# Lapin0t/py-swirld

Hardware: AMD Instinct MI355X
Metric: events/sec through divide_rounds+decide_fame (higher is better)
Workload: dtype int32; 1 GPU; 256 members, 1000000 events, uniform-gossip hashgraph, one batch divide_rounds + decide_fame per step; members=256, events=1000000, seed=3, parallelism=replicas x1 (no data-path collective); the one-hashgraph split is `value_strong`, rounds=284, new_c_last_step=280

## Files before the change

### py-swirld_amd/csrc/swirld_hip.hip

```cpp
#include <hip/hip_runtime.h>

#include <algorithm>
#include <atomic>
#include <chrono>
#include <cstdarg>
#include <cstdio>
#include <cstring>
#include <initializer_list>
#include <string>
#include <thread>
#include <type_traits>
#include <vector>

#include "../../include/swirld_hip.h"
#include "entry_plan.h"
#include "owned.h"
#include "kernels.hip.h"
#define SW_PROV_ROWS 16
#define SW_RANGE_SLOTS 16
#include "crypto.hip.h"
#include "validate.hip.h"
#include "pack.hip.h"
#include "sign.hip.h"
#include "data.hip.h"
#include "exact.hip.h"
#include "batch.hip.h"
#include "ingest.hip.h"
#include "resolve.hip.h"
#include "gossip.hip.h"
#include "walk.hip.h"
#include "wire.hip.h"
#include "turn.hip.h"
#include "consensus.hip.h"
#include "votes.hip.h"

namespace {

std::string g_create_error;

using owned::DBuf;
using owned::Event;
using owned::Pinned;
using owned::Stream;

struct PinnedVec {
    Pinned<int32_t> buf;
    size_t n = 0;
    size_t size() const { return n; }
    int32_t* data() { return buf.p; }
    int32_t& operator[](size_t i) { return buf.p[i]; }
    void clear() { n = 0; }
    bool resize(size_t m) {
        if (m > buf.cap) {
            Pinned<int32_t> q;
            if (!q.reserve(std::max(m, buf.cap + buf.cap / 2 + 4096))) return false;
            if (n) memcpy(q.p, buf.p, n * sizeof(int32_t));
            buf = std::move(q);
        }
        n = m;
        return true;
    }
};

}

struct VmTable {
    bool active = false;
    char* base = nullptr;
    size_t va_bytes = 0, chunk = 0;
    std::vector<hipMemGenericAllocationHandle_t> handle;
// ... 80 lines not shown
    Event ev_payload;
    bool payload_pending = false;
    std::vector<int32_t> seq_h;
    Pinned<SmallRec> h_small;
    Event ev_small;
    bool small_pending = false;
    Pinned<char> h_pin;
    int max_height = 0;
    int64_t N = 0, cap = 0, divided = 0;
    struct IngestState {
        DBuf<int32_t> d_tab;
        DBuf<int32_t> d_hist;
        DBuf<int32_t> d_ht_stat;
        std::vector<int32_t> stage;
        Event ev_ht;
        bool ht_pending = false;
        int64_t ht_first = 0, ht_K = 0;
        int64_t ht_dev_upto = 0;
        int64_t dev_batches = 0, dev_events = 0, fallback = 0, host_ht = 0;
        void rewind() {}
        void reset() { ht_pending = false; ht_dev_upto = 0; }
    } ing;
    struct IdState {
        DBuf<unsigned char> d_id;
        DBuf<int32_t> d_idtab;
        int idtab_log = 0;
        int64_t n_ids = 0;
        DBuf<int32_t> d_idflag;
        DBuf<unsigned char> d_pl;
        DBuf<unsigned char> d_pl_in;
        Pinned<int32_t> h_plcnt;
        int64_t pl_calls = 0, pl_waves = 0, pl_accepted = 0, pl_rebuilds = 0;
        double pl_ms[4] = {0, 0, 0, 0};
        void rewind() {}
        void reset() { n_ids = 0; }
    } ids;
    struct ExportState {
        DBuf<int32_t> d;
        DBuf<unsigned char> d_out;
        int64_t calls = 0, events = 0;
        double ms[2] = {0, 0};
        int lanes = 16;
    } xp;
    struct VotesState {
        DBuf<unsigned char> d_sched, d_plan, d_work, d_out;
        int sched_calls = -1;
        std::vector<unsigned char> sched_stage, plan_stage;
        DBuf<unsigned long long> d_cnt;
        int64_t calls = 0, rows = 0, entries = 0;
        double ms[2] = {0, 0};
        void rewind() { sched_calls = -1; }
        void reset() {}
    } votes;
    struct WalkState {
        DBuf<int32_t> d;
        DBuf<unsigned> d_bits;
        DBuf<int32_t> d_q;
        DBuf<int32_t> d_list;
        DBuf<int32_t> d_trunk;
        DBuf<int32_t> d_children;
        int64_t trunk_N = -1;
        int threads = 1024;
        int64_t calls = 0, events = 0, levels = 0;
        double ms[3] = {0, 0, 0};
        void rewind() {}
        void reset() { trunk_N = -1; }
    } walk;
    struct ConsensusState {
        DBuf<int32_t> d_rr;
        DBuf<double> d_cts;
        DBuf<int32_t> d_tx;
        int64_t tx_len = 0;
        DBuf<int32_t> d_ordpos;
        DBuf<unsigned char> d_out;
        int64_t record_calls = 0, recorded = 0, export_calls = 0, exported = 0;
        void rewind() { tx_len = 0; }
        void reset() {}
    } cons;
    struct ValidateState {
        std::vector<uint8_t> keys, usable;
        DBuf<unsigned char> d_keys;
        DBuf<unsigned char> d_tab;
        DBuf<unsigned char> d_in;
        int64_t calls = 0, events = 0, accepted = 0, builds = 0;
        double ms[2] = {0, 0};
    } val;
    struct PackState {
        std::string mod = "swirld", qual = "Event";
        bool hdr_stale = true;
        std::vector<uint8_t> hdr;
        DBuf<unsigned char> d_hdr;
        DBuf<unsigned char> d;
        DBuf<unsigned char> d_in;
        DBuf<unsigned char> d_out;
        Pinned<int32_t> h_cnt;
        int64_t calls = 0, events = 0, bytes = 0;
        double ms[2] = {0, 0};
    } pack;
    struct DataState {
        DBuf<unsigned char> d_arena;
        DBuf<long long> d_off;
        DBuf<unsigned char> d_none;
        int64_t n_data = 0;
        int64_t used = 0;
        DBuf<unsigned char> d;
        DBuf<unsigned char> d_in;
// ... 86 lines not shown
    int64_t stage_calls = 0;
    DBuf<unsigned long long> d_dbg;
    DBuf<unsigned long long> d_dbg_blk;
    int64_t dbg_iter_base = 0;
    int dbg_minor = 1;
    DBuf<unsigned char> d_small;
    Event ev_aux_done, ev_cs_done, ev_main_mark, ev_bounds, ev_loop_done;
    std::vector<int32_t> divided_cnt;
    std::vector<int32_t> bounds_stage;
    DBuf<int32_t> d_evalround, d_evalpos, d_lo_r, d_cur, d_unres, d_lo_next, d_pos_next, d_farslot, d_force, d_cand, d_gallop;
    DBuf<u64> d_Mb;
    DBuf<int32_t> d_Pc;
    DBuf<int32_t> d_rsc;
    DBuf<u64> d_found64;
    DBuf<unsigned char> d_rb;
    Pinned<unsigned char> h_rb_all;
    std::vector<Event> rb_events;
    RState* d_state = nullptr;
    int* d_flow_err = nullptr;
    struct { int32_t* p = nullptr; } d_front;
    int32_t* d_treecnt = nullptr;
    unsigned* d_prov = nullptr;
    FameCounters* d_fc = nullptr;
    unsigned char* h_rb = nullptr;
    int gate_lag = 0, gate_step = 1;
    int gated = 1;
    int shot_pct = 100, shot_extra = 2;
    size_t rb_bytes = 0;
    Pinned<unsigned char> h_fame;
    std::vector<int32_t> front;
    std::vector<int32_t> front_dev;
    std::vector<int32_t> lo0_h;
    std::vector<unsigned char> cons_h;
    int sw_dirty_from = 1;

    int skip = 1;
    int gallop_after = 2;
    int elect_impl = 1;
    int elect_cg = 128;
    int K = 28;
    int MCAP = 0;
    int NEARCAP = 0;
    int BATCH = 24;
    int cansee_impl = 6;
    int ring_H_req = 0;
    int flow_cfg = 1;
    int tally_impl = 1;
    bool tally_auto = true;
    bool K_auto = true;
    int K_flat = 28;
    int eval_src = 0;
    int band_blocks = 512;
    int fin_blocks = 1024;
    int mid_pct = 0;
    int fin_band = 1;
    int band_fast = 1;
    int tally_filter = 0;
    int tally_pf = 1;

    struct GraphKey { int Rcap; int64_t N; void* lo; void* L; void* chain; void* S; void* round; int K, tally_impl, BATCH, MCAP, variant; };
    bool use_graph = true;
    hipGraph_t loop_graph[4] = {nullptr, nullptr, nullptr, nullptr};
    hipGraphExec_t loop_exec[4] = {nullptr, nullptr, nullptr, nullptr};
    int graph_big = 64;
    GraphKey loop_key{};
    int64_t stat_iters = 0, stat_events = 0;
    int64_t gstat_iters = 0, gstat_events = 0;

    bool profiling = false;
    sw_timings tm{};
    sw_counters ctr{};
    std::vector<Event> ev_pool;
    size_t ev_used = 0;
    PinnedVec transactions;
    std::vector<int32_t> ord_pos;
    std::vector<unsigned char> sig_h;
    std::vector<int32_t> chain_start_h, chain_ev_h;
    DBuf<int32_t> d_q, d_acc_ev, d_acc_ri, d_sorted, d_hostflag;
    DBuf<int32_t> d_ord_rounds, d_fwm, d_ordat, d_rowsum, d_grp;
    DBuf<long long> d_oblk;
    Pinned<char> h_ord;
    std::vector<Event> ord_events;
    Pinned<int32_t> h_ord_stage;
    DBuf<int32_t> d_big_ri, d_sk_ev;
    DBuf<long long> d_big_off;
    DBuf<double> d_sk_ts;
    DBuf<u64> d_sk_k8;
    DBuf<int32_t> d_seg;
    DBuf<int32_t> d_fd;
    DBuf<unsigned char> d_white;
    DBuf<double> d_ts;
    DBuf<double> d_tch;
    DBuf<int> d_err;
    DBuf<u64> d_flow_dbg;
};

namespace {

int fail(sw_ctx* c, int code, const char* fmt, ...) {
    char buf[512];
    va_list ap;
    va_start(ap, fmt);
    vsnprintf(buf, sizeof buf, fmt, ap);
    va_end(ap);
    if (c) c->err = buf; else g_create_error = buf;
    return code;
// ... 776 lines not shown
    for (int g = 0; g < 4; ++g) {
        if (kGraphSizes[g] <= 0) continue;
        while (left >= kGraphSizes[g]) {
            if (!c->loop_exec[g]) {
                HIPCHK(c, hipStreamBeginCapture(c->stream, hipStreamCaptureModeThreadLocal));
                const int64_t launches_before = c->ctr.kernel_launches;
                for (int it = 0; it < kGraphSizes[g]; ++it) enqueue_iteration<NW>(c, it & 1, nullptr);
                c->ctr.kernel_launches = launches_before;
                HIPCHK(c, hipStreamEndCapture(c->stream, &c->loop_graph[g]));
                HIPCHK(c, hipGraphInstantiate(&c->loop_exec[g], c->loop_graph[g], nullptr, nullptr, 0));
            }
            HIPCHK(c, hipGraphLaunch(c->loop_exec[g], c->stream));
            c->ctr.kernel_launches += 2 * kGraphSizes[g];
            left -= kGraphSizes[g];
        }
    }
    return SW_OK;
}

template <int NW>
int launch_finalize(sw_ctx* c, hipStream_t ax, int64_t first, int64_t K, int R, int blocks) {
    const int np = c->npad;
    if (K <= 0) return SW_OK;
    if (!c->fin_band) {
        hipLaunchKernelGGL(k_finalize_events<NW>, dim3((unsigned)std::min<int64_t>((K + 3) / 4, blocks)), dim3(256), 0, ax, (const int*)c->d_L.p,
                           (const int*)c->d_cr.p, (const int*)c->d_lo.p, R, (int)first, (int)K, c->d_round.p, c->d_S.p, np);
        c->ctr.kernel_launches++;
        return SW_OK;
    }
    if (!c->d_fin.p) {
        CHK(dgrow(c, c->d_fin, 4, 0));
        HIPCHK(c, hipMemset(c->d_fin.p, 0, 16));
    }
    HIPCHK(c, hipMemsetAsync(c->d_fin.p, 0, sizeof(unsigned), ax));
    hipLaunchKernelGGL(k_finalize_check, dim3((unsigned)((K + 255) / 256)), dim3(256), 0, ax, (const int*)c->d_cr.p, (const int*)c->d_lo.p, R,
                       (int)first, (int)K, (const int*)c->d_round.p, np, c->d_finlist.p, c->d_fin.p);
    hipLaunchKernelGGL(k_finalize_listed<NW>, dim3((unsigned)std::min<int64_t>((K + 3) / 4, std::min(blocks, 1024))), dim3(256), 0, ax, (const int*)c->d_L.p,
                       (const int*)c->d_cr.p, (const int*)c->d_lo.p, R, (const int*)c->d_finlist.p, c->d_fin.p, c->d_round.p, c->d_S.p, np);
    c->ctr.kernel_launches += 2;
    return SW_OK;
}

inline int predict_shot(const sw_ctx* c, int64_t n_new_events, bool gated = false) {
    int shot = std::min<int64_t>(c->BATCH, 2 + (n_new_events / (12 * (int64_t)c->n) + 1) * 2);
    const int64_t si = gated ? c->gstat_iters : c->stat_iters, se = gated ? c->gstat_events : c->stat_events;
    if (si > 0 && se > 0) {
        const double pred = (double)si / (double)se * (double)n_new_events;
        shot = std::max(2, (int)(pred * c->shot_pct / 100.0) + c->shot_extra);
    }
    return std::min(shot, 4096) & ~1;
}

template <int NW>
int launch_voter_masks(sw_ctx* c, int r0, int R, hipStream_t strm) {
    const int np = c->npad;
    if (R > c->Sw_rows) {
        int nr = c->Sw_rows ? c->Sw_rows : 256;
        while (nr < R) nr *= 2;
        u64* q = nullptr;
        hipError_t e = hipMalloc((void**)&q, (size_t)nr * np * NW * sizeof(u64));
        if (e != hipSuccess) return fail(c, SW_ENOMEM, "hipMalloc(Sw) failed: %s", hipGetErrorString(e));
        poison(q, (size_t)nr * np * NW * sizeof(u64));
        HIPCHK(c, hipStreamSynchronize(c->stream_aux));
        if (c->Sw_rows && c->d_Sw.p)
            HIPCHK(c, hipMemcpy(q, c->d_Sw.p, (size_t)c->Sw_rows * np * NW * sizeof(u64), hipMemcpyDeviceToDevice));
        c->d_Sw.adopt(q, (size_t)nr * np * NW);
        c->Sw_rows = nr;
    }
    r0 = std::max(1, r0);
    if (R <= r0) return SW_OK;
    const uint32_t tot2 = 2u * c->tot;
    const int total = (R - r0) * np;
    if (c->unit_stake && c->tally_impl >= 1)
        hipLaunchKernelGGL(k_voter_masks_bits<NW>, dim3((total + 3) / 4), dim3(256), 0, strm,
                           (const int*)c->d_wit.p, (const int*)c->d_L.p, (const int*)c->d_lo.p, (const uint32_t*)c->d_S.p,
                           tot2, r0, R, np, (uint32_t*)c->d_Sw.p, c->d_fc);
    else if (c->unit_stake)
        hipLaunchKernelGGL((k_voter_masks<NW, true>), dim3((total + 3) / 4), dim3(256), 0, strm,
                           (const int*)c->d_wit.p, (const int*)c->d_L.p, (const int*)c->d_lo.p, (const u64*)c->d_S.p,
                           (const uint32_t*)c->d_stake.p, tot2, r0, R, np, c->d_Sw.p, c->d_fc);
    else
        hipLaunchKernelGGL((k_voter_masks<NW, false>), dim3((total + 3) / 4), dim3(256), 0, strm,
                           (const int*)c->d_wit.p, (const int*)c->d_L.p, (const int*)c->d_lo.p, (const u64*)c->d_S.p,
                           (const uint32_t*)c->d_stake.p, tot2, r0, R, np, c->d_Sw.p, c->d_fc);
    c->ctr.kernel_launches++;
    return SW_OK;
}

struct EdgeHeights {
    std::vector<int64_t> start;
    std::vector<std::vector<int32_t>> h;
    int32_t at(int64_t e) const {
        for (size_t i = 0; i < start.size(); ++i)
            if (e >= start[i] && e < start[i] + (int64_t)h[i].size()) return h[i][(size_t)(e - start[i])];
        return 0;
    }
};

void height_span(const sw_ctx* c, int64_t a, int64_t b, int* hmin, int* hmax, const EdgeHeights& edge) {
    int lo = 0x7fffffff, hi = -1;
    int64_t e = a;
    const int64_t have = (int64_t)c->ht.size();
    while (e < b) {
        if ((e & 4095) == 0 && e + 4096 <= b) {
            lo = std::min(lo, c->blk_hmin[e >> 12]);
            hi = std::max(hi, c->blk_hmax[e >> 12]);
            e += 4096;
        } else {
            const int32_t h = e < have ? c->ht[e] : edge.at(e);
            lo = std::min(lo, h);
            hi = std::max(hi, h);
            ++e;
        }
    }
    *hmin = lo;
    *hmax = hi;
}

int heights_for_spans(sw_ctx* c, const std::vector<int64_t>& cut, EdgeHeights& edge) {
    CHK(heights_ready(c));
    const int64_t have = (int64_t)c->sp.size();
    if (have >= c->N) return SW_OK;
    if (c->ing.ht_dev_upto < c->N) return ensure_dag_h(c);
    for (size_t i = 0; i < cut.size(); ++i) {
        const int64_t x = cut[i];
        const int64_t a = std::max<int64_t>(x & ~(int64_t)4095, have), b = std::min<int64_t>((x | (int64_t)4095) + 1, c->N);
        if ((x & 4095) == 0 || b <= a) continue;
        edge.start.push_back(a);
        edge.h.emplace_back((size_t)(b - a));
        HIPCHK(c, hipMemcpyAsync(edge.h.back().data(), c->d_ht.p + a, (size_t)(b - a) * sizeof(int32_t), hipMemcpyDeviceToHost, c->stream));
    }
    HIPCHK(c, hipStreamSynchronize(c->stream));
    return SW_OK;
}

struct StageClock {
    bool on;
    std::chrono::steady_clock::time_point last;
    explicit StageClock(bool on_) : on(on_) { if (on) last = std::chrono::steady_clock::now(); }
    void mark(double* acc) {
        if (!on) return;
        const auto now = std::chrono::steady_clock::now();
        *acc += std::chrono::duration<double, std::micro>(now - last).count();
        last = now;
    }
};


struct DeferredTail {
    bool armed;
    int i, r_start, R;
    int64_t a0, k0;
    hipEvent_t loop_done;
};

struct DivideCall {
    const int64_t first, K;
    std::vector<int64_t> cut;
    int S = 0;
    bool flow = false;
    bool preswept = false;
    bool gated = false;
    std::vector<int> hmins, nlevs;
    bool bounds_pending = false;
    std::vector<int32_t> clen_prev, clen;
    int64_t fin_from = 0;
    DeferredTail tail{};
    StageClock clk;
    Span sp_total, sp_rl;
    hipEvent_t cs_t0 = nullptr, cs_t1 = nullptr, fin_t0 = nullptr;
    float tally_ms = 0.f;
    int tally_launches = 0;
    std::vector<Span> cansee_spans;
    DivideCall(const sw_ctx* c, int64_t first_, int64_t K_) : first(first_), K(K_), clk(c->debug_timing) {}
};

LoopGate* loop_gate(sw_ctx* c) { return reinterpret_cast<LoopGate*>(c->d_rb.p + SW_GATE_OFF); }

void plan_cuts(const sw_ctx* c, DivideCall& d) {
    const int64_t first = d.first, K = d.K;
    std::vector<int64_t>& cut = d.cut;
    cut.assign(1, first);
    if (const char* cs_ = getenv("SW_CUTS"); cs_ && K >= 65536) {
        for (const char* q = cs_; *q;) {
            char* end = nullptr;
            const double f = strtod(q, &end);
            if (end == q) break;
            const int64_t bnd = ((first + (int64_t)(f * (double)K)) >> 12) << 12;
            if (bnd > cut.back() && bnd < first + K) cut.push_back(bnd);
            q = *end ? end + 1 : end;
        }
    } else if (K >= 65536 && c->pipe > 1) {
        const int64_t head = K / 16;
        const int P = c->pipe;
        double w[SW_PROV_ROWS], tot = 0.0;
        for (int s_ = 0; s_ < P; ++s_) { w[s_] = P < 4 ? 1.0 : (s_ == 0 ? 0.5 : s_ == 1 ? 0.9 : s_ == 2 ? 1.2 : 1.0); tot += w[s_]; }
        double acc = 0.0;
        for (int s_ = 0; s_ < P; ++s_) {
            const int64_t at = head + (int64_t)((double)(K - head) * (acc / tot));
            acc += w[s_];
            const int64_t bnd = ((first + at) >> 12) << 12;
            if (bnd > cut.back() && bnd < first + K) cut.push_back(bnd);
        }
    }
    cut.push_back(first + K);
    d.S = (int)cut.size() - 1;
    d.flow = c->cansee_impl >= 6;
}

void choose_tally(sw_ctx* c, const DivideCall& d) {
    if (!c->tally_auto || !c->unit_stake) return;
    int impl = 1;
    if (c->npad == 256 && c->n > 200 && d.K >= 65536) {
        int32_t lo_ = 0x7fffffff, hi_ = 0;
        for (int m = 0; m < c->n; ++m) { lo_ = std::min(lo_, c->nev[m]); hi_ = std::max(hi_, c->nev[m]); }
// ... 184 lines not shown
    int r_start = 0x7fffffff;
    bool row0_dirty = false;
    std::copy(c->bounds_stage.begin() + (size_t)(i + 1) * np, c->bounds_stage.begin() + (size_t)(i + 2) * np, d.clen.begin());
    for (int m = 0; m < c->n; ++m) {
        if (d.clen[m] > d.clen_prev[m]) {
            if (c->front[m] < 0) {
                c->lo0_h[m] = c->first_ev[m];
                c->front[m] = 0;
                row0_dirty = true;
            }
            r_start = std::min(r_start, c->front[m]);
        }
    }
    *r_start_out = r_start == 0x7fffffff ? std::max(c->R - 1, 0) : r_start;
    HIPCHK(c, hipStreamWaitEvent(c->stream, c->cs_events[i_sweep], 0));
    if (row0_dirty) {
        HIPCHK(c, hipMemcpyAsync(c->d_lo.p, c->lo0_h.data(), np * sizeof(int32_t), hipMemcpyHostToDevice, c->stream));
        std::copy(c->front.begin(), c->front.end(), c->front_dev.begin());
        HIPCHK(c, hipMemcpyAsync(c->d_front.p, c->front_dev.data(), np * sizeof(int32_t), hipMemcpyHostToDevice, c->stream));
    }
    d.clk.mark(&c->stage_us[1]);
    return SW_OK;
}

void chunk_check(sw_ctx* c, int i) {
    const sw_ctx::ChunkPlan& pl = c->chunk_plan[i];
    if (pl.G < 2) return;
    const unsigned* pv = reinterpret_cast<const unsigned*>(c->h_rb + ((unsigned char*)c->d_prov - c->d_rb.p));
    for (int k = 1; k < pl.G; ++k) {
        const unsigned cnt = pv[(size_t)i * SW_MAX_CHUNKS + k];
        const int64_t len = pl.a[k + 1] - pl.a[k];
        c->ctr.chunk_provisional += cnt;
        if (cnt > (unsigned)std::min<int64_t>((len * c->n) / (32 * (c->chunk_cfg == 1 ? 2 : 4)), 0x7fffffff)) {
            c->ctr.chunk_resweeps++;
            c->chunks_off = true;
        }
    }
    c->ctr.chunk_repaired += pv[(size_t)SW_PROV_ROWS * SW_MAX_CHUNKS + i];
}

int after_loop(sw_ctx* c, DivideCall& d, int i, int r_start) {
    d.clk.mark(&c->stage_us[2]);
    HIPCHK(c, hipEventRecord(c->ev_loop_done, c->stream));
    for (int k = d.gated ? 0 : i; k <= i; ++k) chunk_check(c, k);
    for (int m = 0; m < c->n; ++m) c->front[m] = std::max(c->front[m], c->front_dev[m]);
    d.clen_prev.swap(d.clen);
    d.clk.mark(&c->stage_us[3]);
    CHK(ensure_rounds(c, c->R + 2));
    d.tail = DeferredTail{true, i, r_start, c->R, d.fin_from, d.cut[i + 1] - d.fin_from, c->ev_loop_done};
    d.clk.mark(&c->stage_us[4]);
    return SW_OK;
}

template <int NW>
int flush_tail(sw_ctx* c, DivideCall& d) {
    DeferredTail& t = d.tail;
    if (!t.armed) return SW_OK;
    t.armed = false;
    const int np = c->npad;
    hipStream_t ax = c->stream_aux;
    HIPCHK(c, hipStreamWaitEvent(ax, t.loop_done, 0));
    if (t.i == 0 && c->profiling) { d.fin_t0 = next_event(c); (void)hipEventRecord(d.fin_t0, ax); }
    const int blocks = (int)std::min<int64_t>((t.k0 + 3) / 4, t.i == d.S - 1 ? 8192 : c->fin_blocks);
    CHK(launch_finalize<NW>(c, ax, t.a0, t.k0, t.R, blocks));
    const int total = (t.R - t.r_start) * np;
    if (total > 0)
        hipLaunchKernelGGL(k_witness_table, dim3((total + 255) / 256), dim3(256), 0, ax,
                           (const int*)c->d_lo.p, t.R, t.r_start, np, c->d_wit.p);
    c->ctr.kernel_launches += 1;
    return launch_voter_masks<NW>(c, t.r_start, t.R, ax);
}


struct LoopRun {
    RState st{};
    int launched = 0;
    int pieces = 0;
    bool spans = false;
    std::vector<Span> tally_spans, resolve_spans;
    std::chrono::steady_clock::time_point t_wait, t_loop;
    int64_t iters_before = 0;
    double waited_ms() const { return std::chrono::duration<double, std::milli>(t_loop - t_wait).count(); }
    double loop_ms() const { return std::chrono::duration<double, std::milli>(std::chrono::steady_clock::now() - t_loop).count(); }
};

void loop_start(sw_ctx* c, LoopRun& L, bool timed, int r_start, int64_t limit, const int32_t* visible_len, int64_t fin_from, int stages) {
    L.t_wait = std::chrono::steady_clock::now();
    L.iters_before = c->ctr.round_iterations;
    if (timed) (void)hipStreamSynchronize(c->stream);
    L.t_loop = std::chrono::steady_clock::now();
    const int np = c->npad;
    hipLaunchKernelGGL(k_loop_init, dim3(1), dim3(std::min(2 * np, 1024)), 0, c->stream, loop_bufs(c), np, r_start,
                       (int)limit, c->NEARCAP, (const int*)visible_len, c->d_chain_len.p, c->eval_src,
                       (int)std::min<int64_t>(c->fin_band ? fin_from : 0x7fffffff, 0x7fffffff),
                       (int)std::min<int64_t>(c->ctr.round_iterations - c->dbg_iter_base, 0x7fffffff),
                       stages, stages ? (const int*)c->d_bounds.p : (const int*)nullptr, stages ? (const long long*)c->d_cuts.p : (const long long*)nullptr);
    c->eval_src = 0;
    c->ctr.kernel_launches++;
}

unsigned char* rb_slot(sw_ctx* c, int j) { return j < 0 ? c->h_rb : c->h_rb_all.p + (size_t)j * c->rb_bytes; }

template <int NW>
int enqueue_shot(sw_ctx* c, LoopRun& L, int n_it, int j) {
    CHK(launch_iterations<NW>(c, n_it, L.spans ? &L.tally_spans : nullptr, L.spans ? &L.resolve_spans : nullptr));
    L.launched += n_it;
    if (c->split_failed) { c->poisoned = true; return fail(c, SW_EIO, "split round loop: a linked context did not arrive at iteration %lld (sw_split_link: every part calls sw_divide_rounds)", c->split_iter); }
    HIPCHK(c, hipGetLastError());
    HIPCHK(c, hipMemcpyAsync(rb_slot(c, j), c->d_rb.p, c->rb_bytes, hipMemcpyDeviceToHost, c->stream));
    if (j >= 0) HIPCHK(c, hipEventRecord(c->rb_events[j], c->stream));
    return SW_OK;
}

int take_read_back(sw_ctx* c, LoopRun& L, int j) {
    if (j >= 0) HIPCHK(c, hipEventSynchronize(c->rb_events[j]));
    else HIPCHK(c, hipStreamSynchronize(c->stream));
    c->h_rb = rb_slot(c, j);
// ... 56 lines not shown
        for (size_t i = 0; i < L.resolve_spans.size() && (int)i < st.iter; ++i) { c->tm.resolve_ms += span_ms(L.resolve_spans[i]); c->tm.resolve_launches++; }
    }
}

template <int NW>
int run_round_loop(sw_ctx* c, DivideCall& d, int i) {
    const int np = c->npad;
    const int64_t limit = d.cut[i + 1], n_new_events = d.cut[i + 1] - d.cut[i];
    int r_start = 0;
    CHK(begin_loop(c, d, i, i, &r_start));
    const bool dbg_t = c->debug_timing && d.K >= 65536;
    LoopRun L;
    L.spans = c->profiling && !c->split;
    d.fin_from = d.cut[i];
    loop_start(c, L, dbg_t, r_start, limit, c->d_bounds.p + (size_t)(i + 1) * np, d.cut[i], 0);
    int shot = predict_shot(c, n_new_events);
    int rest = 0;
    if (i == d.S - 1 && n_new_events >= 65536 && shot >= 64 && c->mid_pct > 0) {
        const int head = std::max(2, (int)((int64_t)shot * c->mid_pct / 100) & ~1);
        rest = std::max(2, (shot - head) & ~1);
        shot = head;
    }
    for (;;) {
        CHK(ensure_rounds(c, c->R + L.launched + shot + 4));
        CHK(enqueue_shot<NW>(c, L, shot, -1));
        if (L.launched == shot) CHK(flush_tail<NW>(c, d));
        CHK(take_read_back(c, L, -1));
        if (L.st.done) break;
        CHK(check_terminates(c, L, 0));
        if (rest) {
            CHK(flush_tail<NW>(c, d));
            CHK(early_finalize<NW>(c, d, L.st, std::min<int64_t>(L.st.mlo, limit), nullptr));
            shot = rest;
            rest = 0;
        } else
        shot = top_up_shot(L.launched);
    }
    account_loop(c, d, L, n_new_events, false);
    if (dbg_t) {
        const double l = L.loop_ms();
        const int64_t its = c->ctr.round_iterations - L.iters_before;
        fprintf(stderr, "[sw] sub-batch %d: %lld events, waited %.3f ms for the sweep, loop %.3f ms, %lld iterations (%.1f us each)\n",
                i, (long long)n_new_events, L.waited_ms(), l, (long long)its, its ? l * 1e3 / (double)its : 0.0);
    }
    return after_loop(c, d, i, r_start);
}


template <int NW>
int take_piece(sw_ctx* c, DivideCall& d, LoopRun& L, int j) {
    CHK(take_read_back(c, L, j));
    const RState& st = L.st;
    if (!c->fin_band || st.done) return SW_OK;
    return early_finalize<NW>(c, d, st, std::min<int64_t>(std::min(st.mlo, st.N), d.first + d.K), c->rb_events[j]);
}

template <int NW>
int gated_schedule(sw_ctx* c, DivideCall& d, LoopRun& L, int total) {
    const int P = std::min(d.S, SW_PROV_ROWS);
    const int piece = std::max(2, (total / P) & ~1);
    int left = total, j = 0;
    bool taken_last = false;
    for (; left > 0 && j < P; ++j) {
        const int n_it = j == P - 1 ? left : std::min(left, piece);
        CHK(enqueue_shot<NW>(c, L, n_it, j));
        left -= n_it;
        if (j > 0) {
            CHK(take_piece<NW>(c, d, L, j - 1));
            if (L.st.done) { taken_last = true; break; }
        }
    }
    L.pieces = j;
    if (!taken_last) CHK(take_read_back(c, L, j - 1));
    while (!L.st.done) {
        CHK(check_terminates(c, L, total));
        const int shot = top_up_shot(L.launched);
        CHK(ensure_rounds(c, c->R + L.launched + shot + 4));
        CHK(enqueue_shot<NW>(c, L, shot, 0));
        CHK(take_read_back(c, L, 0));
    }
    return SW_OK;
}

template <int NW>
int gated_schedule_lag(sw_ctx* c, DivideCall& d, LoopRun& L, int total) {
    const int lag = c->gate_lag, S = d.S;
    int pub = 1;
    for (int j = 0;; ++j) {
        CHK(check_terminates(c, L, total + (int64_t)lag * S, lag));
        CHK(ensure_rounds(c, c->R + L.launched + lag + 4));
        CHK(enqueue_shot<NW>(c, L, lag, j % SW_PROV_ROWS));
        if (pub < S) {
            const int v = std::min(S, pub + c->gate_step);
            for (int i = pub; i < v; ++i) HIPCHK(c, hipStreamWaitEvent(c->stream, c->cs_events[i], 0));
            hipLaunchKernelGGL(k_set_stage, dim3(1), dim3(64), 0, c->stream, loop_gate(c), v);
            c->ctr.kernel_launches++;
            pub = v;
        }
        if (j > 0) {
            CHK(take_piece<NW>(c, d, L, (j - 1) % SW_PROV_ROWS));
            L.pieces = j;
            if (L.st.done) return SW_OK;
        }
    }
}

template <int NW>
int run_gated(sw_ctx* c, DivideCall& d) {
    const int np = c->npad, S = d.S;
    int r_start = 0;
    CHK(begin_loop(c, d, S - 1, 0, &r_start));
    LoopRun L;
    L.spans = c->profiling;
    d.fin_from = d.first;
    loop_start(c, L, c->debug_timing, r_start, d.cut[1], c->d_bounds.p + np, d.first, S);
    const int total = predict_shot(c, d.K, true);
    CHK(ensure_rounds(c, c->R + total + 8));
    if (c->gate_lag > 0) CHK(gated_schedule_lag<NW>(c, d, L, total));
    else CHK(gated_schedule<NW>(c, d, L, total));
    account_loop(c, d, L, d.K, true);
    if (c->debug_timing) {
        fprintf(stderr, "[sw] gated loop: %d sub-batches, %lld events, waited %.3f ms for the first sweep, loop %.3f ms, %lld iterations + %d waiting, %d launched in %d pieces\n",
                S, (long long)d.K, L.waited_ms(), L.loop_ms(), (long long)(c->ctr.round_iterations - L.iters_before - L.st.idle), L.st.idle, L.launched, L.pieces);
    }
    return after_loop(c, d, S - 1, r_start);
}

int finish_call(sw_ctx* c, DivideCall& d) {
    const int np = c->npad, S = d.S, R = c->R;
    const int64_t first = d.first, K = d.K;
    hipEvent_t fin_t1 = nullptr;
    if (c->profiling) { fin_t1 = next_event(c); (void)hipEventRecord(fin_t1, c->stream_aux); }
    HIPCHK(c, hipEventRecord(c->ev_aux_done, c->stream_aux));
    HIPCHK(c, hipEventRecord(c->ev_cs_done, c->stream_cs));
    HIPCHK(c, hipStreamWaitEvent(c->stream, c->ev_aux_done, 0));
    HIPCHK(c, hipStreamWaitEvent(c->stream, c->ev_cs_done, 0));
    span_end(c, d.sp_total);
    if (c->profiling || c->debug_timing) {
        HIPCHK(c, hipStreamSynchronize(c->stream_aux));
        HIPCHK(c, hipStreamSynchronize(c->stream));
        HIPCHK(c, hipStreamSynchronize(c->stream_cs));
    }
    HIPCHK(c, hipGetLastError());
    std::copy(c->bounds_stage.begin() + (size_t)S * np, c->bounds_stage.begin() + (size_t)(S + 1) * np, c->divided_cnt.begin());
    d.clk.mark(&c->stage_us[5]);
    c->sw_dirty_from = std::max(R, 1);
    if (first + K == c->N) std::copy(c->head.begin(), c->head.end(), c->divided_head.begin());
    else for (int64_t e = first; e < first + K; ++e) c->divided_head[c->cr[e]] = (int32_t)e;
    c->divided = first + K;
    c->ctr.events_divided += K;
    c->ctr.rounds = R;
    if (c->profiling) {
        float ms = 0.f;
        if (d.cs_t0 && d.cs_t1) (void)hipEventElapsedTime(&ms, d.cs_t0, d.cs_t1);
        c->tm.can_see_ms = ms;
        c->tm.rounds_ms = span_ms(d.sp_rl);
        c->tm.tally_ms = d.tally_ms;
        c->tm.tally_launches = d.tally_launches;
        { float fm = 0.f; if (d.fin_t0 && fin_t1) (void)hipEventElapsedTime(&fm, d.fin_t0, fin_t1); c->tm.finalize_ms = fm; }
        c->tm.total_ms = span_ms(d.sp_total);
        c->tm.cansee_kernel_ms = 0.f;
        c->tm.cansee_launches = (int32_t)d.cansee_spans.size();
        for (const Span& s_ : d.cansee_spans) c->tm.cansee_kernel_ms += span_ms(s_);
    }
    return SW_OK;
}

template <int NW>
int do_divide(sw_ctx* c, int64_t first, int64_t K) {
    const int np = c->npad;
    c->ev_used = 0;
    DivideCall d(c, first, K);
    c->stage_calls += 1;
    d.sp_total = span_begin(c);
    plan_cuts(c, d);
    choose_tally(c, d);
    CHK(test_preswept(c, d));
    CHK(size_level_tables(c, d));
    CHK(open_sweep_stream(c, d));
    CHK(build_bounds(c, d));
    CHK(plan_chunks(c, d));
    CHK(enqueue_sweeps<NW>(c, d));
    d.clk.mark(&c->stage_us[0]);

    if (d.bounds_pending) HIPCHK(c, hipEventSynchronize(c->ev_bounds));
    CHK(ensure_rounds(c, std::max(c->R, 1) + c->BATCH + 4));
    d.sp_rl = span_begin(c);
    d.clen_prev.assign(c->bounds_stage.begin(), c->bounds_stage.begin() + np);
    d.clen.assign(np, 0);
    if (d.gated) CHK(run_gated<NW>(c, d));
    else for (int i = 0; i < d.S; ++i) CHK(run_round_loop<NW>(c, d, i));
    CHK(flush_tail<NW>(c, d));
    span_end(c, d.sp_rl);
    return finish_call(c, d);
}

int first_undecided_round(const sw_ctx* c) {
    int max_c = 0;
    while (max_c < c->R && c->cons_h[max_c]) ++max_c;
    return max_c;
}

template <int NW>
int fame_launch(sw_ctx* c, int max_c, int part, int nparts, Span* sp_el) {
    const int np = c->npad, R = c->R;
    if (c->payload_pending) HIPCHK(c, hipStreamWaitEvent(c->stream, c->ev_payload, 0));
    const uint32_t tot2 = 2u * c->tot;
    if (c->sw_dirty_from < R || R > c->Sw_rows) CHK(launch_voter_masks<NW>(c, std::min(c->sw_dirty_from, R), R, c->stream));
    c->sw_dirty_from = std::max(R, 1);
    const bool tiled = NW >= 2 && c->elect_impl == 1;
    if (tiled) CHK(dgrow(c, c->d_rsc, (size_t)3 * c->Rcap, 0));
    hipLaunchKernelGGL(k_fame_prep, dim3(std::max(1, std::min(64, (3 * R + 255) / 256))), dim3(256), 0, c->stream, c->d_newc.p + sizeof(FameCounters), R,
                       tiled ? c->d_rsc.p : nullptr, tiled ? 3 * R : 0);
    const int nblk = R - max_c - part > 0 ? (R - max_c - part + nparts - 1) / nparts : 0;
    const int call_idx = (int)c->fame_calls.size();
    if (sp_el) *sp_el = span_begin(c);
    if (nblk > 0) {
        bool split_done = false;
#define SW_ELECT_ARGS (const int*)c->d_wit.p, (const u64*)c->d_Sw.p, (const unsigned char*)c->d_coin.p, (const uint32_t*)c->d_stake.p, \
                      tot2, c->coin_period, max_c, R, np, c->d_fam.p, c->d_cons.p, c->d_newc.p + sizeof(FameCounters), c->d_fc, c->d_dec_call.p, c->d_dec_by.p, call_idx, part, nparts
        if constexpr (NW >= 2) {
            if (c->elect_impl == 1) {
#define SW_ELECT_TILED(CG_)                                                                                                             \
    do {                                                                                                                                \
        if (c->unit_stake) hipLaunchKernelGGL((k_elections_tiled<NW, true, CG_>), dim3(nblk * (64 * NW / (CG_))), dim3((CG_) * NW), 0, c->stream, SW_ELECT_ARGS, c->d_rsc.p);  \
// ... 740 lines not shown
    int nw = 1;
    while (nw * 64 < n_members) nw *= 2;
    c->nw = nw;
    c->npad = nw * 64;
    c->coin_period = coin_period;
    c->device = device;
    c->unit_stake = unit;
    c->tot = (uint32_t)tot;
    c->stake_h.assign(c->npad, 0);
    for (int i = 0; i < n_members; ++i) c->stake_h[i] = (uint32_t)stake[i];
    c->head.assign(n_members, -1);
    c->first_ev.assign(n_members, -1);
    c->front.assign(n_members, -1);
    c->front_dev.assign(c->npad, -1);
    c->divided_head.assign(c->npad, -1);
    c->ord_pos.assign(n_members, 0);
    c->lo0_h.assign(c->npad, SW_INF);
    c->NEARCAP = std::max(64 * c->npad, 4096);
    c->MCAP = std::max(1024 * c->npad, 65536);
    if (c->npad > 512) {
        c->K = 12;
        c->skip = 10;
    }
    std::string knob_err;
    auto knob = [&](const char* name, long long lo, long long hi, auto* dst) {
        const char* s = getenv(name);
        if (!s || !*s) return;
        char* end = nullptr;
        const long long v = strtoll(s, &end, 10);
        if (*end != 0 || v < lo || v > hi) {
            if (knob_err.empty()) { char b[160]; snprintf(b, sizeof b, "%s=%s: an integer in [%lld, %lld]", name, s, lo, hi); knob_err = b; }
            return;
        }
        *dst = static_cast<std::remove_pointer_t<decltype(dst)>>(v);
    };
    int graph = c->use_graph ? 1 : 0;
    c->K_auto = !(getenv("SW_TALLY_K") && *getenv("SW_TALLY_K"));
    c->tally_auto = !(getenv("SW_TALLY_IMPL") && *getenv("SW_TALLY_IMPL"));
    knob("SW_TALLY_K", 1, 63, &c->K);
    knob("SW_BAND", 64, 1 << 28, &c->NEARCAP);
    knob("SW_BAND_MAX", 64, 1 << 28, &c->MCAP);
    c->MCAP = std::max(c->MCAP, c->NEARCAP);
    knob("SW_BATCH", 1, 4096, &c->BATCH);
    knob("SW_GRAPH", 0, 1, &graph);
    knob("SW_GRAPH_BIG", 0, 512, &c->graph_big);
    c->graph_big &= ~1;
    c->use_graph = graph != 0;
    if (c->npad >= 1024) c->band_blocks = 256;
    knob("SW_BAND_BLOCKS", 1, 4096, &c->band_blocks);
    knob("SW_TALLY_PF", 0, 1, &c->tally_pf);
    knob("SW_MID_PCT", 0, 99, &c->mid_pct);
    knob("SW_FIN_BAND", 0, 1, &c->fin_band);
    knob("SW_FIN_BLOCKS", 64, 8192, &c->fin_blocks);
    if (c->npad > 512) c->pipe = 1;
    knob("SW_PIPE", 1, SW_PROV_ROWS - 1, &c->pipe);
    if (c->npad > 256) c->cansee_impl = 3;
    knob("SW_CANSEE_IMPL", 2, 6, &c->cansee_impl);
    if (c->cansee_impl == 4 || c->cansee_impl == 5) knob_err = "SW_CANSEE_IMPL: 6 (dataflow sweep), 2 or 3 (level-bucketed sweep)";
    knob("SW_TALLY_IMPL", 0, 2, &c->tally_impl);
    knob("SW_FLOW_CFG", 0, 3, &c->flow_cfg);
    knob("SW_CHUNKS", 1, SW_MAX_CHUNKS, &c->chunks);
    knob("SW_CHUNK_CFG", 0, 2, &c->chunk_cfg);
    knob("SW_BAND_FAST", 0, 1, &c->band_fast);
    if (c->npad > 256) c->tally_filter = 1;
    knob("SW_TALLY_FILTER", 0, 1, &c->tally_filter);
    knob("SW_SPLIT_EMULATE", 0, SW_MAX_PARTS, &c->split_emulate);
    knob("SW_SHOT_PCT", 10, 400, &c->shot_pct);
    knob("SW_GATED", 0, 1, &c->gated);
    knob("SW_GATE_LAG", 0, 256, &c->gate_lag);
    knob("SW_GATE_STEP", 1, SW_PROV_ROWS, &c->gate_step);
    if (c->gate_lag & 1) knob_err = "SW_GATE_LAG: an even number in [0, 256] (iteration parity)";
    knob("SW_SHOT_EXTRA", 0, 64, &c->shot_extra);
    knob("SW_CHUNK_MIN", 64, 1 << 30, &c->chunk_min);
    c->halo = 32 * (int64_t)c->npad;
    knob("SW_HALO", 0, 1 << 24, &c->halo);
    knob("SW_ELECT_IMPL", 0, 1, &c->elect_impl);
    knob("SW_ELECT_CG", 64, 256, &c->elect_cg);
    if (c->elect_cg != 64 && c->elect_cg != 128 && c->elect_cg != 256) knob_err = "SW_ELECT_CG: 64, 128 or 256";
    knob("SW_GALLOP", 0, 255, &c->gallop_after);
    knob("SW_SKIP", 0, 32, &c->skip);
    knob("SW_RING_H", 0, 64, &c->ring_H_req);
    if (!knob_err.empty()) {
        delete c;
        return fail(nullptr, SW_EINVAL, "%s", knob_err.c_str());
    }
    auto debug_buf = [&](auto& b, size_t words) {
        if (dgrow(c, b, words, 0) == SW_OK) (void)hipMemset(b.p, 0, words * 8);
        else { (void)hipGetLastError(); c->err.clear(); }
    };
    c->debug_timing = getenv("SW_DEBUG_TIMING") != nullptr;
    if (c->debug_timing) {
        debug_buf(c->d_flow_dbg, 8);
    }
    if (const char* e_ = getenv("SW_EXPORT_LANES")) { const int g = atoi(e_); if (g == 4 || g == 8) c->xp.lanes = g; }
    if (const char* e_ = getenv("SW_WALK_THREADS")) { const int w = atoi(e_); if (w >= 64 && w <= wlk::MAX_THREADS && w % 64 == 0) c->walk.threads = w; }
    if (const char* e_ = getenv("SW_WIRE_BLOCKS")) { const int w = atoi(e_); if (w >= 1 && w <= 4096) c->wire.blocks = w; }
    history_knobs(c);
    if (getenv("SW_DEBUG_CLOCKS")) {
        c->dbg_minor = atoi(getenv("SW_DEBUG_CLOCKS")) >= 2 ? 0 : 1;
        if (atoi(getenv("SW_DEBUG_CLOCKS")) == 3) {
            debug_buf(c->d_dbg_blk, (size_t)SW_DBG_MAX_ITERS * 2 * 2048);
        }
        debug_buf(c->d_dbg, (size_t)SW_DBG_MAX_ITERS * 32);
    }
    c->nev.assign(n_members, 0);
    c->BATCH = (c->BATCH + 1) & ~1;
// ... 1337 lines not shown
    }
    if (evictions) *evictions = c->vm.evictions;
    return SW_OK;
}

int sw_set_forks(sw_ctx* c, int accept) {
    if (!c) return SW_EINVAL;
    if (accept != 0 && accept != 1) return fail(c, SW_EINVAL, "sw_set_forks: 0 (refuse) or 1 (accept)");
    c->forks_mode = accept;
    return SW_OK;
}

int sw_get_exact(sw_ctx* c, int* out) {
    if (!c || !out) return SW_EINVAL;
    *out = c->exact ? 1 : 0;
    return SW_OK;
}

int sw_get_witness_order(sw_ctx* c, int r, int32_t* members, int* n_out) {
    if (!c || !members || !n_out) return SW_EINVAL;
    *n_out = 0;
    if (r < 0 || r >= c->R) return fail(c, SW_ERANGE, "round %d outside [0, %d)", r, c->R);
    HIPCHK(c, hipSetDevice(c->device));
    const int np = c->npad, n = c->n;
    if (c->exact) {
        int32_t cnt = 0;
        std::vector<int32_t> row(np);
        HIPCHK(c, hipMemcpyAsync(&cnt, c->ex.wcnt.p + r, sizeof cnt, hipMemcpyDeviceToHost, c->stream));
        HIPCHK(c, hipMemcpyAsync(row.data(), c->ex.worder.p + (size_t)r * np, np * sizeof(int32_t), hipMemcpyDeviceToHost, c->stream));
        HIPCHK(c, hipStreamSynchronize(c->stream));
        for (int i = 0; i < cnt; ++i) members[i] = row[i];
        *n_out = cnt;
        return SW_OK;
    }
    std::vector<int32_t> row(np);
    HIPCHK(c, hipMemcpyAsync(row.data(), c->d_wit.p + (size_t)r * np, np * sizeof(int32_t), hipMemcpyDeviceToHost, c->stream));
    HIPCHK(c, hipStreamSynchronize(c->stream));
    std::vector<std::pair<int32_t, int32_t>> ws;
    for (int m = 0; m < n; ++m) if (row[m] >= 0) ws.push_back({row[m], m});
    std::sort(ws.begin(), ws.end());
    for (size_t i = 0; i < ws.size(); ++i) members[i] = ws[i].second;
    *n_out = (int)ws.size();
    return SW_OK;
}

int sw_rewind(sw_ctx* c) {
    if (!c) return SW_EINVAL;
    HIPCHK(c, hipSetDevice(c->device));
    HIPCHK(c, hipStreamSynchronize(c->stream_cs));
    HIPCHK(c, hipStreamSynchronize(c->stream_aux));
    const size_t rows = (size_t)c->Rcap * c->npad;
    c->hist.rewind();
    c->votes.rewind();
    c->ing.rewind();
    c->ids.rewind();
    c->data.rewind();
    c->walk.rewind();
    c->fame_calls.clear();
    c->votes_partial = false;
    c->eval_src = 0;
    std::fill(c->cons_call.begin(), c->cons_call.end(), -1);
    {
        RewindJob J{};
        int nj = 0;
        auto job = [&](void* p_, size_t words, int v) { if (p_ && words) { J.p[nj] = (int*)p_; J.n[nj] = words; J.v[nj] = v; ++nj; } };
        job(c->d_lo.p, rows, SW_INF);
        job(c->d_lopos.p, rows, 0);
        job(c->d_wit.p, rows, -1);
        job(c->d_dec_call.p, rows, -1);
        job(c->d_dec_by.p, rows, -1);
        job(c->d_evalround.p, 2 * (size_t)c->npad, -1);
        job(c->d_evalpos.p, 2 * (size_t)c->npad, 0);
        job(c->d_front.p, c->npad, -1);
        job(c->d_round.p, (size_t)c->N, -1);
        if (rows % 4 == 0) job(c->d_fam.p, rows / 4, -1);
        else HIPCHK(c, hipMemsetAsync(c->d_fam.p, 0xff, rows, c->stream));
        if (c->Rcap % 4 == 0) job(c->d_cons.p, (size_t)c->Rcap / 4, 0);
        else HIPCHK(c, hipMemsetAsync(c->d_cons.p, 0, c->Rcap, c->stream));
        size_t longest = 1;
        for (int i = 0; i < nj; ++i) longest = std::max<size_t>(longest, J.n[i]);
        if (nj) {
            hipLaunchKernelGGL(k_rewind_fill, dim3((unsigned)std::min<size_t>((longest + 1023) / 1024, 1024), nj), dim3(256), 0, c->stream, J);
            c->ctr.kernel_launches++;
            HIPCHK(c, hipGetLastError());
        }
    }
    std::fill(c->front.begin(), c->front.end(), -1);
    std::fill(c->divided_cnt.begin(), c->divided_cnt.end(), 0);
    std::fill(c->lapsed.begin(), c->lapsed.end(), 0);
    if (c->vm.active && c->vm.lo > 0) {
        HIPCHK(c, hipDeviceSynchronize());
        VmTable& v = c->vm;
        void* base = nullptr;
        hipError_t e = hipMemAddressReserve(&base, v.va_bytes, 0, nullptr, 0);
        if (e != hipSuccess) { c->poisoned = true; return fail(c, SW_ENOMEM, "hipMemAddressReserve failed on rewind: %s", hipGetErrorString(e)); }
        for (size_t s_ = 0; s_ < v.mapped.size(); ++s_)
            if (v.mapped[s_]) { HIPCHK(c, hipMemUnmap(v.base + s_ * v.chunk, v.chunk)); v.pool.push_back(v.handle[s_]); v.mapped[s_] = 0; }
        HIPCHK(c, hipMemAddressFree(v.base, v.va_bytes));
        CHK(vm_flush_translations(c));
        v.base = (char*)base;
        v.lo = 0; v.hi = 0;
        c->vm_scratch_ok = false;
        c->d_L.alias((int32_t*)base, c->d_L.cap);
        c->first_resident = 0;
        CHK(vm_ensure(c, (size_t)c->N * c->npad * sizeof(int32_t)));
    }
    c->ranges.clear();
    c->present.clear();
    std::fill(c->divided_head.begin(), c->divided_head.end(), -1);
    std::fill(c->lo0_h.begin(), c->lo0_h.end(), SW_INF);
    std::fill(c->cons_h.begin(), c->cons_h.end(), 0);
    c->divided = 0;
    c->R = 0;
    c->sw_dirty_from = 1;
    c->dbg_iter_base = c->ctr.round_iterations;
    c->transactions.clear();
    c->cons.rewind();
    std::fill(c->ord_pos.begin(), c->ord_pos.end(), 0);
    if (c->exact) CHK(exact_rewind(c));
    return SW_OK;
}

int sw_reset(sw_ctx* c) {
    if (!c) return SW_EINVAL;
    CHK(sw_rewind(c));
    c->cr.clear(); c->sp.clear(); c->op.clear(); c->ht.clear(); c->seq_h.clear();
    std::fill(c->head.begin(), c->head.end(), -1);
    std::fill(c->first_ev.begin(), c->first_ev.end(), -1);
    std::fill(c->nev.begin(), c->nev.end(), 0);
    c->blk_hmin.clear(); c->blk_hmax.clear();
    c->max_height = 0;
    c->N = 0;
    c->sig_h.clear();
    c->chain_cap.clear();
    c->chain_ev_h.clear();
    c->pool_used = 0;
    c->pool_h_valid = true;
    if (c->stream_io) HIPCHK(c, hipStreamSynchronize(c->stream_io));
    c->payload_pending = false;
    c->hist.reset();
    c->votes.reset();
    c->cons.reset();
    c->ing.reset();
    c->ids.reset();
    c->data.reset();
    c->walk.reset();
    if (c->ids.idtab_log) HIPCHK(c, hipMemsetAsync(c->ids.d_idtab.p, 0xff, sizeof(int32_t) << c->ids.idtab_log, c->stream));
    c->exact = false;
    c->chunks_off = false;
    return SW_OK;
}

int sw_split_link(sw_ctx* const* ctxs, int parts) {
    if (!ctxs || parts < 2 || parts > SW_MAX_PARTS) return fail(nullptr, SW_EINVAL, "sw_split_link: 2 .. %d contexts", SW_MAX_PARTS);
    sw_ctx* c0 = ctxs[0];
    for (int q = 0; q < parts; ++q) {
        sw_ctx* c = ctxs[q];
        if (!c) return fail(c0, SW_EINVAL, "sw_split_link: context %d is NULL", q);
        for (int o = 0; o < q; ++o) if (ctxs[o] == c) return fail(c, SW_EINVAL, "sw_split_link: context %d given twice", q);
        if (c->poisoned) return fail(c, SW_EIO, "context poisoned by an earlier failure");
        if (c->split) return fail(c, SW_EINVAL, "sw_split_link: context %d is linked already", q);
        if (c->exact || c->vm.active || !c->unit_stake)
            return fail(c, SW_ENOTSUP, "sw_split_link: unit stake, the fast path and the plain can_see table only");
        if (c->n != c0->n || c->N != c0->N || c->divided != c0->divided || c->R != c0->R || c->coin_period != c0->coin_period)
            return fail(c, SW_EINVAL, "sw_split_link: context %d does not hold the same hashgraph, divided to the same point, as context 0", q);
        if (c->MCAP != c0->MCAP || c->NEARCAP != c0->NEARCAP || c->skip != c0->skip || c->gallop_after != c0->gallop_after || c->pipe != c0->pipe)
            return fail(c, SW_EINVAL, "sw_split_link: context %d was created under other tuning knobs than context 0", q);
    }
    SplitGroup* g = new SplitGroup();
    g->parts = parts;
    for (int w = 0; w < 2; ++w) for (int q = 0; q < SW_MAX_PARTS; ++q) g->rec[w][q].store(0);
    for (int q = 0; q < parts; ++q) {
        sw_ctx* c = ctxs[q];
        g->ctx[q] = c;
        if (hipSetDevice(c->device) != hipSuccess) { split_dissolve(g); return fail(c0, SW_EIO, "hipSetDevice(%d) failed", c->device); }
        for (int o = 0; o < parts; ++o)
            if (ctxs[o]->device != c->device) {
                int can = 0;
                (void)hipDeviceCanAccessPeer(&can, c->device, ctxs[o]->device);
                if (!can) { split_dissolve(g); return fail(c0, SW_ENOTSUP, "sw_split_link: device %d cannot map the memory of device %d", c->device, ctxs[o]->device); }
                const hipError_t e = hipDeviceEnablePeerAccess(ctxs[o]->device, 0);
                if (e != hipSuccess && e != hipErrorPeerAccessAlreadyEnabled) { (void)hipGetLastError(); split_dissolve(g); return fail(c0, SW_EIO, "hipDeviceEnablePeerAccess failed: %s", hipGetErrorString(e)); }
                (void)hipGetLastError();
            }
        for (int w = 0; w < 2; ++w)
            for (auto& e : g->ev[w][q])
                if (hipEventCreateWithFlags(&e, hipEventDisableTiming) != hipSuccess) { split_dissolve(g); return fail(c0, SW_EIO, "hipEventCreate failed"); }
    }
    for (int q = 0; q < parts; ++q) {
        sw_ctx* c = ctxs[q];
        c->split_saved[0] = c->tally_impl; c->split_saved[1] = c->tally_auto; c->split_saved[2] = c->K; c->split_saved[3] = c->K_auto;
        c->tally_impl = 1; c->tally_auto = false; c->K = c->K_flat; c->K_auto = false;
        c->split_part = q;
        c->split_iter = 0;
// ... 3237 lines not shown
```

Before: 172.4 million events/s.

## Build witness table and voter masks piecewise beside the divide loop

Adds a piecewise tail that, after each early-finalize step, computes on the aux stream which rounds are safely settled. It then builds the witness table and voter bit-masks for those rounds while the main round-division loop is still running. The final flush only covers the remaining rounds, so less of this tail work sits after the loop. The cost is an extra small range-scan kernel per early finalize and device-side range bookkeeping. There is also a risk of races if the safety predicate is wrong.

```diff
diff --git a/py-swirld_amd/csrc/swirld_hip.hip b/py-swirld_amd/csrc/swirld_hip.hip
--- a/py-swirld_amd/csrc/swirld_hip.hip
+++ b/py-swirld_amd/csrc/swirld_hip.hip
@@ -16,6 +16,7 @@
 #include "entry_plan.h"
 #include "owned.h"
 #include "kernels.hip.h"
+#include "tail.hip.h"
 #define SW_PROV_ROWS 16
 #define SW_RANGE_SLOTS 16
 #include "crypto.hip.h"
@@ -202,6 +203,14 @@
         void rewind() { sched_calls = -1; }
         void reset() {}
     } votes;
+    struct TailState {
+        DBuf<int32_t> d_words;
+        bool started = false;
+        int launches = 0, r_start = 0;
+        void begin_call(int r_start_) { started = false; launches = 0; r_start = r_start_; }
+        void rewind() { begin_call(0); }
+        void reset() {}
+    } tail;
     struct WalkState {
         DBuf<int32_t> d;
         DBuf<unsigned> d_bits;
@@ -394,6 +403,8 @@
     int eval_src = 0;
     int band_blocks = 512;
     int fin_blocks = 1024;
+    int piece_tail = 1;
+    int tail_blocks = 256;
     int mid_pct = 0;
     int fin_band = 1;
     int band_fast = 1;
@@ -1276,7 +1287,7 @@
 }
 
 template <int NW>
-int launch_voter_masks(sw_ctx* c, int r0, int R, hipStream_t strm) {
+int ensure_Sw(sw_ctx* c, int R) {
     const int np = c->npad;
     if (R > c->Sw_rows) {
         int nr = c->Sw_rows ? c->Sw_rows : 256;
@@ -1291,11 +1302,20 @@
         c->d_Sw.adopt(q, (size_t)nr * np * NW);
         c->Sw_rows = nr;
     }
+    return SW_OK;
+}
+
+inline bool masks_are_bits(const sw_ctx* c) { return c->unit_stake && c->tally_impl >= 1; }
+
+template <int NW>
+int launch_voter_masks(sw_ctx* c, int r0, int R, hipStream_t strm) {
+    const int np = c->npad;
+    CHK(ensure_Sw<NW>(c, R));
     r0 = std::max(1, r0);
     if (R <= r0) return SW_OK;
     const uint32_t tot2 = 2u * c->tot;
     const int total = (R - r0) * np;
-    if (c->unit_stake && c->tally_impl >= 1)
+    if (masks_are_bits(c))
         hipLaunchKernelGGL(k_voter_masks_bits<NW>, dim3((total + 3) / 4), dim3(256), 0, strm,
                            (const int*)c->d_wit.p, (const int*)c->d_L.p, (const int*)c->d_lo.p, (const uint32_t*)c->d_S.p,
                            tot2, r0, R, np, (uint32_t*)c->d_Sw.p, c->d_fc);
@@ -1385,6 +1405,7 @@
     bool flow = false;
     bool preswept = false;
     bool gated = false;
+    bool piece_tail = false;
     std::vector<int> hmins, nlevs;
     bool bounds_pending = false;
     std::vector<int32_t> clen_prev, clen;
@@ -1675,6 +1696,35 @@
     return SW_OK;
 }
 
+
+template <int NW>
+int launch_tail_ranged(sw_ctx* c, int bound, int final_R, int final_from, int blocks) {
+    if (bound <= 0) return SW_OK;
+    const int np = c->npad;
+    hipStream_t ax = c->stream_aux;
+    const int64_t total = (int64_t)bound * np;
+    const int* words = c->tail.d_words.p;
+    hipLaunchKernelGGL(k_witness_table_ranged, dim3((unsigned)std::min<int64_t>((total + 255) / 256, blocks)), dim3(256), 0, ax,
+                       (const int*)c->d_lo.p, words, final_R, final_from, np, c->d_wit.p);
+    hipLaunchKernelGGL(k_voter_masks_bits_ranged<NW>, dim3((unsigned)std::min<int64_t>((total + 3) / 4, blocks)), dim3(256), 0, ax,
+                       (const int*)c->d_wit.p, (const int*)c->d_L.p, (const int*)c->d_lo.p, (const uint32_t*)c->d_S.p,
+                       2u * c->tot, words, final_R, final_from, np, (uint32_t*)c->d_Sw.p);
+    c->ctr.kernel_launches += 2;
+    return SW_OK;
+}
+
+template <int NW>
+int piece_tail(sw_ctx* c, DivideCall& d, const RState& st) {
+    sw_ctx::TailState& t = c->tail;
+    CHK(ensure_Sw<NW>(c, st.r + 1));
+    hipLaunchKernelGGL(k_tail_range, dim3(1), dim3(256), 0, c->stream_aux, (const int*)c->d_lo.p, c->npad, st.r,
+                       (int)std::min<int64_t>(d.fin_from, 0x7fffffff), t.started ? -1 : t.r_start, t.d_words.p);
+    c->ctr.kernel_launches++;
+    t.started = true;
+    t.launches++;
+    return launch_tail_ranged<NW>(c, st.r - t.r_start, -1, -1, c->tail_blocks);
+}
+
 template <int NW>
 int flush_tail(sw_ctx* c, DivideCall& d) {
     DeferredTail& t = d.tail;
@@ -1686,6 +1736,10 @@
     if (t.i == 0 && c->profiling) { d.fin_t0 = next_event(c); (void)hipEventRecord(d.fin_t0, ax); }
     const int blocks = (int)std::min<int64_t>((t.k0 + 3) / 4, t.i == d.S - 1 ? 8192 : c->fin_blocks);
     CHK(launch_finalize<NW>(c, ax, t.a0, t.k0, t.R, blocks));
+    if (d.piece_tail) {
+        CHK(ensure_Sw<NW>(c, t.R));
+        return launch_tail_ranged<NW>(c, t.R - t.r_start, t.R, c->tail.started ? -1 : t.r_start, 2048);
+    }
     const int total = (t.R - t.r_start) * np;
     if (total > 0)
         hipLaunchKernelGGL(k_witness_table, dim3((total + 255) / 256), dim3(256), 0, ax,
@@ -1848,7 +1902,10 @@
     CHK(take_read_back(c, L, j));
     const RState& st = L.st;
     if (!c->fin_band || st.done) return SW_OK;
-    return early_finalize<NW>(c, d, st, std::min<int64_t>(std::min(st.mlo, st.N), d.first + d.K), c->rb_events[j]);
+    const int64_t fin_before = d.fin_from;
+    CHK(early_finalize<NW>(c, d, st, std::min<int64_t>(std::min(st.mlo, st.N), d.first + d.K), c->rb_events[j]));
+    if (d.piece_tail && d.fin_from > fin_before) CHK(piece_tail<NW>(c, d, st));
+    return SW_OK;
 }
 
 template <int NW>
@@ -1906,6 +1963,9 @@
     const int np = c->npad, S = d.S;
     int r_start = 0;
     CHK(begin_loop(c, d, S - 1, 0, &r_start));
+    d.piece_tail = c->piece_tail && c->fin_band && masks_are_bits(c);
+    c->tail.begin_call(r_start);
+    if (d.piece_tail) CHK(dgrow(c, c->tail.d_words, 2, 0));
     LoopRun L;
     L.spans = c->profiling;
     d.fin_from = d.first;
@@ -1938,6 +1998,12 @@
         HIPCHK(c, hipStreamSynchronize(c->stream_cs));
     }
     HIPCHK(c, hipGetLastError());
+    if (c->debug_timing && d.piece_tail) {
+        int32_t w[2] = {c->tail.r_start, c->tail.r_start};
+        if (c->tail.started) HIPCHK(c, hipMemcpy(w, c->tail.d_words.p, sizeof w, hipMemcpyDeviceToHost));
+        fprintf(stderr, "[sw] piece tail: %d launches beside the loop took the rounds [%d, %d), the tail behind it [%d, %d)\n",
+                c->tail.launches, c->tail.r_start, w[1], w[1], R);
+    }
     std::copy(c->bounds_stage.begin() + (size_t)S * np, c->bounds_stage.begin() + (size_t)(S + 1) * np, c->divided_cnt.begin());
     d.clk.mark(&c->stage_us[5]);
     c->sw_dirty_from = std::max(R, 1);
@@ -1967,6 +2033,7 @@
     const int np = c->npad;
     c->ev_used = 0;
     DivideCall d(c, first, K);
+    c->tail.begin_call(0);
     c->stage_calls += 1;
     d.sp_total = span_begin(c);
     plan_cuts(c, d);
@@ -2813,6 +2880,8 @@
     knob("SW_MID_PCT", 0, 99, &c->mid_pct);
     knob("SW_FIN_BAND", 0, 1, &c->fin_band);
     knob("SW_FIN_BLOCKS", 64, 8192, &c->fin_blocks);
+    knob("SW_PIECE_TAIL", 0, 1, &c->piece_tail);
+    knob("SW_TAIL_BLOCKS", 16, 8192, &c->tail_blocks);
     if (c->npad > 512) c->pipe = 1;
     knob("SW_PIPE", 1, SW_PROV_ROWS - 1, &c->pipe);
     if (c->npad > 256) c->cansee_impl = 3;
@@ -4256,6 +4325,7 @@
     const size_t rows = (size_t)c->Rcap * c->npad;
     c->hist.rewind();
     c->votes.rewind();
+    c->tail.rewind();
     c->ing.rewind();
     c->ids.rewind();
     c->data.rewind();
@@ -4344,6 +4414,7 @@
     c->payload_pending = false;
     c->hist.reset();
     c->votes.reset();
+    c->tail.reset();
     c->cons.reset();
     c->ing.reset();
     c->ids.reset();
diff --git a/py-swirld_amd/csrc/tail.hip.h b/py-swirld_amd/csrc/tail.hip.h
--- /dev/null
+++ b/py-swirld_amd/csrc/tail.hip.h
@@ -0,0 +1,90 @@
+#pragma once
+
+#include "tail_range.h"
+
+#define SW_TAIL_CHUNK 1024
+
+__global__ void __launch_bounds__(256)
+k_tail_range(const int* __restrict__ lo, int npad, int r_committed, int fin_upto, int first_done, int* words) {
+    __shared__ int s_max[SW_TAIL_CHUNK + 1];
+    const int lane = lane_id();
+    const int wave = threadIdx.x >> 6, nwaves = blockDim.x >> 6;
+    const int done = first_done >= 0 ? first_done : words[1];
+    const int top = min(r_committed, done + SW_TAIL_CHUNK - 1);
+    for (int r = done + wave; r <= top; r += nwaves) {
+        int mx = -1;
+        for (int m = lane; m < npad; m += 64) mx = max(mx, tail::finite(lo[(size_t)r * npad + m]));
+        mx = wave_max_i32(mx);
+        if (lane == 0) s_max[r - done] = mx;
+    }
+    __syncthreads();
+    if (threadIdx.x == 0) {
+        words[0] = done;
+        words[1] = tail::safe_upto([&](int r) { return s_max[r - done]; }, done, top, fin_upto);
+    }
+}
+
+__device__ __forceinline__ void tail_rounds(const int* __restrict__ words, int final_R, int final_from, int* r0, int* r1) {
+    if (final_R >= 0) { *r0 = final_from >= 0 ? final_from : words[1]; *r1 = final_R; }
+    else { *r0 = words[0]; *r1 = words[1]; }
+}
+
+__global__ void __launch_bounds__(256)
+k_witness_table_ranged(const int* __restrict__ lo, const int* __restrict__ words, int final_R, int final_from, int npad, int* wit) {
+    int r0, r1;
+    tail_rounds(words, final_R, final_from, &r0, &r1);
+    const int total = (r1 - r0) * npad;
+    for (int i = blockIdx.x * blockDim.x + threadIdx.x; i < total; i += gridDim.x * blockDim.x) {
+        const int r = r0 + i / npad, c = i % npad;
+        const int a = lo[(size_t)r * npad + c];
+        const int b = lo[(size_t)(r + 1) * npad + c];
+        wit[(size_t)r * npad + c] = (a != SW_INF && b > a) ? a : -1;
+    }
+}
+
+template <int NW>
+__global__ void __launch_bounds__(256)
+k_voter_masks_bits_ranged(const int* __restrict__ wit, const int* __restrict__ L, const int* __restrict__ lo,
+                          const uint32_t* __restrict__ S32, uint32_t tot2, const int* __restrict__ words, int final_R, int final_from,
+                          int npad, uint32_t* Sw32) {
+    constexpr int W32 = 2 * NW, PLT = ilog2_c(64 * NW) + 1;
+    __shared__ int s_pk[4][64 * NW];
+    const int lane = lane_id();
+    const int wib = threadIdx.x >> 6;
+    int r0, r1;
+    tail_rounds(words, final_R, final_from, &r0, &r1);
+    r0 = max(r0, 1);
+    const int total = (r1 - r0) * npad;
+    int* pk = s_pk[wib];
+    for (int wv = blockIdx.x * 4 + wib; wv < total; wv += gridDim.x * 4) {
+        const int r = r0 + wv / npad, c = wv % npad;
+        const int y = wit[(size_t)r * npad + c];
+        uint32_t* out = Sw32 + ((size_t)r * npad + c) * W32;
+        if (y < 0) {
+            if (lane < W32) out[lane] = 0;
+            continue;
+        }
+        u64 ex[NW];
+#pragma unroll
+        for (int j = 0; j < NW; ++j) {
+            const int col = j * 64 + lane;
+            const int k = L[(size_t)y * npad + col];
+            const bool valid = k >= lo[(size_t)(r - 1) * npad + col] && k < lo[(size_t)r * npad + col];
+            pk[col] = valid ? k : -1;
+            ex[j] = __ballot(wit[(size_t)(r - 1) * npad + col] >= 0);
+        }
+        __builtin_amdgcn_fence(__ATOMIC_ACQ_REL, "wavefront");
+        __builtin_amdgcn_wave_barrier();
+        uint32_t b[PLT];
+        bits_accumulate<NW>(pk, S32, b, lane);
+        const uint32_t gt = bits_finish<NW>(b, tot2 / 3u);
+        const int w = lane % W32;
+        uint32_t exw = 0;
+#pragma unroll
+        for (int j = 0; j < NW; ++j)
+            if ((w >> 1) == j) exw = (uint32_t)(ex[j] >> (32 * (w & 1)));
+        if (lane < W32) out[w] = gt & exw;
+        __builtin_amdgcn_fence(__ATOMIC_ACQ_REL, "wavefront");
+        __builtin_amdgcn_wave_barrier();
+    }
+}
diff --git a/py-swirld_amd/csrc/tail_range.h b/py-swirld_amd/csrc/tail_range.h
--- /dev/null
+++ b/py-swirld_amd/csrc/tail_range.h
@@ -0,0 +1,30 @@
+#pragma once
+
+#if defined(__HIPCC__)
+#define TAIL_HD __host__ __device__
+#else
+#define TAIL_HD
+#endif
+
+namespace tail {
+
+constexpr int INF = 0x7fffffff;
+
+TAIL_HD inline int finite(int v) { return v == INF ? -1 : v; }
+
+TAIL_HD inline int row_max(const int* row, int npad) {
+    int mx = -1;
+    for (int m = 0; m < npad; ++m) { const int v = finite(row[m]); mx = v > mx ? v : mx; }
+    return mx;
+}
+
+TAIL_HD inline bool round_safe(int max_this, int max_next, int fin_upto) { return max_next <= fin_upto && max_this < fin_upto; }
+
+template <class RowMax>
+TAIL_HD inline int safe_upto(RowMax rowmax, int done_upto, int r_committed, int fin_upto) {
+    int p = done_upto < 0 ? 0 : done_upto;
+    while (p <= r_committed - 1 && round_safe(rowmax(p), rowmax(p + 1), fin_upto)) ++p;
+    return p;
+}
+
+}
```

Measured after the change: 173.6 million events/s, median of 3. No clear change (+0.7%).
